# google/layered-scene-inference

Measured on AMD Instinct MI355X. Metric: rendered views/sec (BxLxHxW splat+warp), higher is better.
Workload: dtype f32; 1 GPU; cfg3: 4-layer LDI 256x768, batch 32 per GPU (32 total), trg_downsampling 0.5, kitti cameras, compose_layers, smooth disparities; launch=graph, input_sets_rotated=3, parallelism=batch-sharded replicas x1 (no collective)

## Files before the change

include/lsi_hip.h:

```cpp
#ifndef LSI_HIP_H_
#define LSI_HIP_H_

#include <stddef.h>
#include <stdint.h>

#ifdef __cplusplus
extern "C" {
#endif

#define LSI_VERSION 100

#define LSI_OK 0
#define LSI_EINVAL -1
#define LSI_ENULL -2
#define LSI_EWORKSPACE -3
#define LSI_ELAUNCH -4
#define LSI_EUNSUPPORTED -5

#define LSI_COMPOSE 1u
#define LSI_WANT_DISP 2u
#define LSI_HAS_MASK 4u
#define LSI_WS_KEEP 8u
#define LSI_DETERMINISTIC 16u

// ... 423 lines not shown
#define LSI_FC_X_F32 2u
#define LSI_FC_OUT_F32 4u
typedef struct LsiFcDesc {
  int32_t M, K, N;
  int32_t groups;
  int32_t taps;
  uint32_t flags;
  int64_t w_sn, w_sk;
  int64_t tap_off[4];
  float eps;
  int32_t reserved;
} LsiFcDesc;
size_t lsi_fc_desc_bytes(void);
int lsi_fc_supported(const LsiFcDesc* d);
size_t lsi_fc_workspace_bytes(const LsiFcDesc* d);
int lsi_fc_fwd(const LsiFcDesc* d, const void* x, const float* w, const float* beta, void* y,
               float* z, float* mean_rstd, void* workspace, size_t workspace_bytes,
               lsi_stream_t stream);
int lsi_fc_bwd(const LsiFcDesc* d, const void* x, const float* w, const void* dy,
               const void* y, const float* z, const float* mean_rstd, void* dx, float* dw,
               float* dbeta, void* workspace, size_t workspace_bytes, lsi_stream_t stream);

#define LSI_IMAGE_MAX_PIXELS 16843009
typedef struct LsiImageDesc {
  int64_t offset;
  int32_t H, W, C;
  int32_t reserved;
} LsiImageDesc;
int lsi_area_resize_u8(int32_t n, const LsiImageDesc* desc_host,
                       const LsiImageDesc* desc_dev, const uint8_t* packed,
                       size_t packed_bytes, int32_t Ho, int32_t Wo, int32_t Co,
                       float* out, lsi_stream_t stream);

#ifdef __cplusplus
}
#endif
#endif
```

layered-scene-inference_amd/build.py:

```python
import os
import shutil
import subprocess
import sys

PKG = os.path.dirname(os.path.abspath(__file__))
ROOT = os.path.dirname(PKG)
CSRC = os.path.join(PKG, 'csrc')
SO = os.path.join(PKG, 'liblsi_hip.so')
SOURCES = ['lsi_splat.hip', 'lsi_splat_stream.hip', 'lsi_splat_stream2.hip',
           'lsi_splat_tile.hip', 'lsi_splat_bwd_stream.hip',
           'lsi_splat_sweep.hip',
           'lsi_sampling.hip', 'lsi_loss.hip', 'lsi_eval.hip', 'lsi_bn.hip', 'lsi_host.hip', 'lsi_conv.hip',
           'lsi_conv_wgrad.hip', 'lsi_conv_igemm.hip', 'lsi_conv_wgrad_igemm.hip',
           'lsi_conv_first.hip', 'lsi_conv_f32.hip', 'lsi_scene.hip', 'lsi_fc.hip',
           'lsi_image.hip', 'lsi_ssim.hip', 'lsi_edge_smooth.hip']
HEADERS = [os.path.join(CSRC, 'lsi_common.h'),
           os.path.join(CSRC, 'lsi_layers.h'),
           os.path.join(CSRC, 'lsi_reduce.h'),
           os.path.join(CSRC, 'lsi_splat_internal.h'),
           os.path.join(CSRC, 'lsi_bn_ws.h'),
           os.path.join(CSRC, 'lsi_conv_host.h'),
           os.path.join(CSRC, 'lsi_conv_device.h'),
           os.path.join(ROOT, 'include', 'lsi_hip.h')]

HIPCC_FLAGS = [
    '--offload-arch=gfx950', '-O3', '-std=c++17', '-fPIC',
    '-ffp-contract=off',
    '-munsafe-fp-atomics',
    '-fno-fast-math', '-Wall', '-Wno-unused-function',
]


def hipcc():
  exe = shutil.which('hipcc') or '/opt/rocm/bin/hipcc'
  if not os.path.exists(exe):
    raise RuntimeError('hipcc not found; ROCm toolchain is required')
  return exe


def _stale(target, deps):
  if not os.path.exists(target):
    return True
  t = os.path.getmtime(target)
  return any(os.path.getmtime(d) > t for d in deps)


SO_HOOKS = os.path.join(PKG, 'liblsi_hip_hooks.so')
LAST_BUILD = {}
# ... 41 lines not shown
```

layered-scene-inference_amd/lsi/_C.py:

```python
import ctypes
import os

import torch

_PKG = os.path.dirname(os.path.dirname(os.path.abspath(__file__)))
SO_PATH = os.path.join(_PKG, 'liblsi_hip_%s.so' % os.environ['LSI_HIP_LIB'] if
                       os.environ.get('LSI_HIP_LIB') else 'liblsi_hip.so')

LSI_OK = 0
LSI_COMPOSE, LSI_WANT_DISP, LSI_HAS_MASK, LSI_WS_KEEP = 1, 2, 4, 8
LSI_DETERMINISTIC = 16
LSI_PACKED_RGBD = 32
LSI_GRAD_M = 64
LSI_PATH_AUTO, LSI_PATH_ATOMIC, LSI_PATH_ROWBAND, LSI_PATH_STREAM = 0, 1, 2, 3
LSI_PATH_TILE = 4
LSI_SCENE_IMG, LSI_SCENE_DISP, LSI_SCENE_IMG_ROOM, LSI_SCENE_DISP_ROOM = 1, 2, 4, 8
LSI_SCENE_MAX_PLANES = 16
LSI_FC_BN, LSI_FC_X_F32, LSI_FC_OUT_F32 = 1, 2, 4
LSI_IMAGE_MAX_PIXELS = 16843009
PATH_NAMES = {1: 'atomic', 2: 'rowband', 3: 'stream', 4: 'tile'}

_c_f = ctypes.POINTER(ctypes.c_float)
_c_i = ctypes.POINTER(ctypes.c_int32)

# ... 40 lines not shown


class LsiEdgeSmoothDesc(ctypes.Structure):
  _fields_ = (
      [(n, ctypes.c_int32) for n in ('L', 'B', 'H', 'W', 'order', 'normalise')] +
      [(n, ctypes.c_int64) for n in ('d_sl', 'd_sb', 'd_sy', 'd_sx',
                                     'g_sl', 'g_sb', 'g_sy', 'g_sx', 'g_sc')] +
      [(n, ctypes.c_float) for n in ('alpha', 'eps')])


class LsiConvDesc(ctypes.Structure):
  _fields_ = [(n, ctypes.c_int32) for n in (
      'N', 'H', 'W', 'Cin', 'OH', 'OW', 'Cout', 'KH', 'KW', 'stride', 'pad_t', 'pad_l')]


class LsiSceneDesc(ctypes.Structure):
  _fields_ = ([(n, ctypes.c_int32) for n in ('B', 'V', 'P', 'Hs', 'Ws', 'H', 'W',
                                             'n_box', 'soft')] +
              [('min_disp', ctypes.c_float), ('temp', ctypes.c_float),
               ('outputs', ctypes.c_uint32)])


class LsiFcDesc(ctypes.Structure):
  _fields_ = ([(n, ctypes.c_int32) for n in ('M', 'K', 'N', 'groups', 'taps')] +
              [('flags', ctypes.c_uint32), ('w_sn', ctypes.c_int64),
               ('w_sk', ctypes.c_int64), ('tap_off', ctypes.c_int64 * 4),
               ('eps', ctypes.c_float), ('reserved', ctypes.c_int32)])


class LsiPackJob(ctypes.Structure):
  _fields_ = ([('w', ctypes.c_void_p), ('dst', ctypes.c_void_p)] +
              [(n, ctypes.c_int32) for n in ('D0', 'D1', 'khw', 'tr', 'ntaps', 'block0')] +
              [('tap', ctypes.c_int8 * 56)])


class LsiConvIO(ctypes.Structure):
  _fields_ = ([(n, ctypes.c_void_p) for n in ('x', 'x2', 'packed', 'out', 'out2',
                                              'bn_workspace', 'workspace')] +
              [('workspace_bytes', ctypes.c_size_t), ('c1', ctypes.c_int32),
               ('groups', ctypes.c_int32)])


class LsiImageDesc(ctypes.Structure):
  _fields_ = ([('offset', ctypes.c_int64)] +
              [(n, ctypes.c_int32) for n in ('H', 'W', 'C', 'reserved')])


_I32, _I64, _VP, _SZ = ctypes.c_int32, ctypes.c_int64, ctypes.c_void_p, ctypes.c_size_t
_DP = ctypes.POINTER(LsiSplatDesc)
_LP = ctypes.POINTER(LsiLossDesc)
_CP = ctypes.POINTER(LsiConvDesc)
_F32 = ctypes.c_float
SIGNATURES = {
    'lsi_version': (ctypes.c_int, []),
    'lsi_strerror': (ctypes.c_char_p, [ctypes.c_int]),
    'lsi_bg_weight': (ctypes.c_float, [ctypes.c_double] * 3),
    'lsi_rowband_ok': (ctypes.c_int, [_DP, _VP]),
    'lsi_stream_ok': (ctypes.c_int, [_DP, _VP]),
    'lsi_splat_workspace_bytes': (_SZ, [_DP]),
    'lsi_stream_adapt_state': (ctypes.c_int, [ctypes.POINTER(LsiStreamAdapt)]),
    'lsi_splat_fwd': (ctypes.c_int, [_DP] + [_VP] * 8 + [_SZ, _VP]),
    'lsi_splat_bwd_workspace_bytes': (_SZ, [_DP]),
    'lsi_splat_bwd': (ctypes.c_int, [_DP] + [_VP] * 12 + [_SZ, _VP]),
    'lsi_splat_bwd_m': (ctypes.c_int, [_DP] + [_VP] * 13 + [_SZ, _VP]),
    'lsi_splat_bwd_disp_workspace_bytes': (_SZ, [_DP]),
    'lsi_splat_bwd_disp': (ctypes.c_int, [_DP] + [_VP] * 15 + [_SZ, _VP]),
# ... 68 lines not shown
    'lsi_conv2d_bwd_data_cat': (ctypes.c_int, [_CP, _VP, _VP, _VP, _VP, _I32, _VP]),
    'lsi_conv2d_wgrad_cat': (ctypes.c_int, [_CP, _VP, _VP, _I32, _VP, _VP, _I32, _VP, _SZ, _VP]),
    'lsi_conv2d_workspace_bytes': (_SZ, [_CP, _I32]),
    'lsi_conv2d_run': (ctypes.c_int, [_CP, _I32, ctypes.POINTER(LsiConvIO), _VP]),
    'lsi_conv2d_wgrad_workspace_bytes': (_SZ, [_CP]),
    'lsi_conv2d_wgrad': (ctypes.c_int, [_CP] + [_VP] * 4 + [_SZ, _VP]),
    'lsi_conv2d_first_supported': (ctypes.c_int, [_CP]),
    'lsi_conv2d_first_fwd': (ctypes.c_int, [_CP, _VP, _I32, _VP, _I32, _VP, _VP, _I32, _VP]),
    'lsi_conv2d_first_wgrad_workspace_bytes': (_SZ, [_CP]),
    'lsi_conv2d_first_wgrad': (ctypes.c_int, [_CP, _VP, _I32, _VP, _VP, _I32, _VP, _SZ, _VP]),
    'lsi_conv2d_f32_supported': (ctypes.c_int, [_CP]),
    'lsi_conv2d_f32_packed_bytes': (_SZ, [_CP]),
    'lsi_conv2d_f32_pack': (ctypes.c_int, [_CP, _I32, _VP, _VP, _SZ, _VP]),
    'lsi_conv2d_f32_pack_job': (ctypes.c_int, [_CP, _I32, _VP, _VP, _SZ,
                                               ctypes.POINTER(LsiPackJob), _c_i]),
    'lsi_conv2d_f32_pack_many': (ctypes.c_int, [_VP, _I32, _I32, _VP]),
    'lsi_conv2d_f32_workspace_bytes': (_SZ, [_CP, _I32]),
    'lsi_conv2d_f32_run': (ctypes.c_int, [_CP, _I32, ctypes.POINTER(LsiConvIO), _VP]),
    'lsi_conv2d_wgrad_f32_workspace_bytes': (_SZ, [_CP]),
    'lsi_conv2d_wgrad_f32': (ctypes.c_int, [_CP, _VP, _VP, _I32, _VP, _VP, _I32, _VP, _SZ,
                                            _VP]),
    'lsi_bn_workspace_floats': (_SZ, [_I64, _I32, _I32, _I32]),
    'lsi_bn_relu_fwd': (ctypes.c_int, [_VP] * 5 + [_I64, _I32, _I32, _I32, _F32, _I32, _VP]),
    'lsi_bn_relu_bwd': (ctypes.c_int, [_VP] * 7 + [_I64, _I32, _I32, _I32, _I32, _VP]),
    'lsi_bn_relu_norm': (ctypes.c_int, [_VP] * 5 + [_I64, _I32, _I32, _I32, _F32, _I32, _VP]),
    'lsi_bn_stats_discard': (ctypes.c_int, [_VP, _I32, _VP]),
    'lsi_fc_desc_bytes': (_SZ, []),
    'lsi_fc_supported': (ctypes.c_int, [ctypes.POINTER(LsiFcDesc)]),
    'lsi_fc_workspace_bytes': (_SZ, [ctypes.POINTER(LsiFcDesc)]),
    'lsi_fc_fwd': (ctypes.c_int, [ctypes.POINTER(LsiFcDesc)] + [_VP] * 7 + [_SZ, _VP]),
    'lsi_fc_bwd': (ctypes.c_int, [ctypes.POINTER(LsiFcDesc)] + [_VP] * 10 + [_SZ, _VP]),
    'lsi_area_resize_u8': (ctypes.c_int, [_I32, _VP, _VP, _VP, _SZ] + [_I32] * 3 +
                           [_VP, _VP]),
}

_lib = None


def lib():
  global _lib
  if _lib is None:
    if not os.path.exists(SO_PATH):
      raise RuntimeError(
          'liblsi_hip.so is missing (%s). Build it with '
          '`python layered-scene-inference_amd/build.py`; there is no CPU or '
          'PyTorch fallback for the lsi HIP ops.' % SO_PATH)
    handle = ctypes.CDLL(SO_PATH)
    for name, (res, args) in SIGNATURES.items():
      fn = getattr(handle, name)
      fn.restype = res
      fn.argtypes = args
    _lib = handle
  return _lib


def check(rc, what):
  if rc != LSI_OK:
    msg = lib().lsi_strerror(rc).decode()
    raise RuntimeError('%s failed: %s (code %d)' % (what, msg, rc))


def require_device(*tensors):
  dev = None
  for t in tensors:
    if t is None:
      continue
# ... 34 lines not shown
```

layered-scene-inference_amd/lsi/nnutils/_hip_conv.py:

```python
import os
import torch

from lsi import _C


def supported(x, cin, cout, k, stride, pred):
  if not (x.is_cuda and x.dim() == 4 and x.dtype == torch.bfloat16):
    return False
  if k != 3 or stride != 1 or cin != 32 or x.shape[1] != 32 or x.shape[3] % 16:
    return False
  if pred:
    if not 1 <= cout <= 4:
      return False
  elif cout not in (16, 32):
    return False
  return (x.is_contiguous(memory_format=torch.channels_last) and
          x.data_ptr() % 16 == 0)


def _launch(x, weight, cout, mode, bias=None):
  n, _, h, w = x.shape
  dev = x.device
  weight = _f32(weight)
  if mode == 1:
# ... 314 lines not shown

_PACKED = {}
_PACK_TABLE = {}


def _pack_layout(w):
  if w.dtype == torch.float32:
    if w.is_contiguous():
      return 0
    if w.dim() == 4 and w.is_contiguous(memory_format=torch.channels_last):
      return 2
  return None


def _pack_source(weight):
  w = weight.detach()
  cl = _pack_layout(w)
  if cl is None:
    return w.float().contiguous(), 0
  return w, cl


_HOOK = [None]
PACK_CHECK = int(os.environ.get('LSI_PACK_CHECK', '0'))
_CHECK_CALLS = [0]


def _install_optimizer_hook():
  if _HOOK[0] is None:
    from torch.optim.optimizer import register_optimizer_step_post_hook
    _HOOK[0] = register_optimizer_step_post_hook(_after_optimizer_step)


def _after_optimizer_step(optimizer, args, kwargs):
  del args, kwargs
  if not _PACKED:
    return
  owned = set()
  for group in optimizer.param_groups:
    for p in group['params']:
      owned.add(id(p))
  if any(k[0] in owned for k in _PACKED):
    repack_all(_owned=owned)


def _packed(desc, mode, weight, training=False, dtype=torch.bfloat16):
  key = (id(weight), mode, dtype)
  hit = _PACKED.get(key)
  training = training and weight.requires_grad
  if training:
    _install_optimizer_hook()
  if training and not (hit is not None and hit.managed):
    _PACKED.pop((id(weight), 1 - mode, dtype), None)
    hit_ok = False
  else:
    hit_ok = True
  geo = (desc.Cin, desc.Cout, desc.KH, desc.KW, desc.stride, desc.pad_t, desc.pad_l)
  if hit is not None and hit.wref() is weight and hit.buf.device == weight.device:
    if hit_ok and hit.version == weight._version and hit.geo == geo:
      if PACK_CHECK and hit.managed:
        _CHECK_CALLS[0] += 1
        if _CHECK_CALLS[0] % PACK_CHECK == 0:
          _verify_pack(hit, weight)
      return hit.buf
  lib = _C.lib()
  dev = weight.device
  p = _PRECISIONS[dtype]
  esz = p.esz
  nbytes = getattr(lib, p.packed_bytes)(ctypes.byref(desc))
  if (hit is not None and hit.wref() is weight and hit.buf.device == dev and
      hit.buf.numel() * esz == nbytes and hit.geo == geo):
    buf = hit.buf
  else:
    buf = torch.empty((nbytes // esz,), dtype=dtype, device=dev)
  src, cl = _pack_source(weight)
  rc = getattr(lib, p.pack)(ctypes.byref(desc), mode | cl, _C.ptr(src), _C.ptr(buf),
                            nbytes, _C.stream_ptr(dev))
  _C.check(rc, p.pack)
  e = _Pack()
  e.wref = weakref.ref(weight, lambda _r, k=key: _PACKED.pop(k, None))
  e.version = weight._version
  e.geo = geo
  e.buf, e.mode, e.desc = buf, mode, desc
  e.dtype = dtype
  e.managed = False
  _PACKED[key] = e
  return buf


def _verify_pack(e, weight):
  src, cl = _pack_source(weight)
  fresh = torch.empty_like(e.buf)
  pack = _PRECISIONS[e.dtype].pack
  rc = getattr(_C.lib(), pack)(ctypes.byref(e.desc), e.mode | cl, _C.ptr(src), _C.ptr(fresh),
                               fresh.numel() * fresh.element_size(), _C.stream_ptr(weight.device))
  _C.check(rc, pack)
  if not torch.equal(fresh, e.buf):
    raise RuntimeError('stale packed weights: a %s parameter was updated behind the '
                       'optimiser hook and the version counter (a write through .data?); '
                       'call _hip_conv.repack_all() after such updates'
                       % (tuple(weight.shape),))


def repack_all(device=None, _owned=None):
  if not _PACKED:
    return 0
  lib = _C.lib()
  by_dev = {}
  for k, e in list(_PACKED.items()):
    w = e.wref()
    if w is None:
      continue
    if _owned is not None and k[0] not in _owned:
      continue
    if not w.is_cuda or _pack_layout(w) is None:
      if device is None or w.device == device:
        _PACKED.pop(k, None)
      continue
    if device is not None and w.device != device:
      continue
    if not w.requires_grad and e.version == w._version:
      continue
    by_dev.setdefault((w.device.index, e.dtype), []).append((e, w))
  n = 0
  for (idx, dtype), items in by_dev.items():
    p = _PRECISIONS[dtype]
    key = tuple((w.data_ptr(), e.buf.data_ptr(), e.mode) for e, w in items)
    tabs = _PACK_TABLE.setdefault(idx if dtype == torch.bfloat16 else (idx, dtype), {})
    tab = tabs.get(key)
    if tab is None:
      jobs = (_C.LsiPackJob * len(items))()
      nb = ctypes.c_int32(0)
      blocks = 0
      for j, (e, w) in enumerate(items):
        rc = getattr(lib, p.pack_job)(ctypes.byref(e.desc), e.mode | _pack_layout(w), w.data_ptr(),
                                  e.buf.data_ptr(), e.buf.numel() * e.buf.element_size(),
                                  ctypes.byref(jobs[j]), ctypes.byref(nb))
        _C.check(rc, p.pack_job)
        jobs[j].block0 = blocks
        blocks += nb.value
      host = torch.frombuffer(bytearray(bytes(jobs)), dtype=torch.uint8)
      tab = (key, host.to(items[0][1].device), len(items), blocks)
      tabs[key] = tab
    dev = items[0][1].device
    with torch.cuda.device(dev):
      rc = getattr(lib, p.pack_many)(tab[1].data_ptr(), tab[2], tab[3], _C.stream_ptr(dev))
# ... 363 lines not shown
```

layered-scene-inference_amd/lsi/nnutils/train_utils.py:

```python
import glob
import json
import os
import time

import torch


def define_default_flags(parser):
  a = parser.add_argument
  a('--checkpoint_dir', default='cachedir/snapshots/')
  a('--pretrain_name', default='')
  a('--pretrain_iter', type=int, default=100000)
  a('--batch_size', type=int, default=2)
  a('--num_iter', type=int, default=100000)
  a('--img_height', type=int, default=256)
  a('--img_width', type=int, default=256)
  a('--log_freq', type=int, default=5)
  a('--checkpoint_freq', type=int, default=50000)
  a('--save_latest_freq', type=int, default=2000)
  a('--learning_rate', type=float, default=0.0001)
  a('--beta1', type=float, default=0.9)
  return parser


# ... 28 lines not shown
    use_gpu = torch.cuda.is_available() and not getattr(opts, 'cpu', False)
    if use_gpu:
      torch.cuda.set_device(self.local_rank)
      self.device = torch.device('cuda', self.local_rank)
      torch.backends.cudnn.benchmark = bool(getattr(opts, 'miopen_search', False))
      if getattr(opts, 'miopen_tune', False):
        os.environ.setdefault('MIOPEN_FIND_ENFORCE', '3')
    if self.world > 1 or (getattr(opts, 'flat_grads', False) and
                          'RANK' in os.environ and 'MASTER_ADDR' in os.environ):
      import torch.distributed as dist
      if not dist.is_initialized():
        dist.init_process_group(backend or ('nccl' if use_gpu else 'gloo'))
      self.dist = dist
    torch.manual_seed(0)
    self.define_data_loader()
    self.model = self.build_model().to(self.device)
    if getattr(opts, 'channels_last', False):
      self.model = self.model.to(memory_format=torch.channels_last)
      if use_gpu:
        from lsi.nnutils import nets
        nets.own_kernel_param_layouts(self.model)
    self.train_model = self.model
    self.use_graph = bool(getattr(opts, 'hip_graph', False)) and use_gpu
    self.flat_grads = bool(getattr(opts, 'flat_grads', False)) or \
        (self.use_graph and self.world > 1)
    if self.world > 1 and not self.flat_grads:
      from torch.nn.parallel import DistributedDataParallel as DDP
      self.train_model = DDP(
          self.model, device_ids=[self.local_rank] if use_gpu else None,
          bucket_cap_mb=25, gradient_as_bucket_view=True)
    self._graph, self._graph_plan, self._static = None, None, None
    self._graph_b = None
    self._graph_warm = 0
    self.optim = torch.optim.Adam(self.model.parameters(),
                                  lr=opts.learning_rate,
                                  betas=(opts.beta1, 0.999), eps=1e-8,
                                  capturable=self.use_graph,
                                  fused=bool(use_gpu) and bool(getattr(opts, 'fused_adam', True)))
    if self.use_graph:
      self._stream = torch.cuda.Stream(self.device)
    if use_gpu:
      from lsi.nnutils import _hip_conv
      env = os.environ.get('LSI_WGRAD_STREAM', '')
      _hip_conv.enable_wgrad_stream(
          self.world == 1 and not self.flat_grads and
          (env == '1' or (env != '0' and not self.use_graph)))
      from lsi.nnutils import nets
      env = os.environ.get('LSI_HEAD_STREAMS', '')
      nets.enable_head_streams(
          self.world == 1 and not self.flat_grads and
          (env == '1' or (env != '0' and not self.use_graph)))
      if getattr(opts, 'fp32_convs', None) is not None:
        nets.F32_CONV = opts.fp32_convs == 'own'
    self.resume()
    if self.flat_grads:
      self._setup_flat_grads()

  def _setup_flat_grads(self):
    params = [p for p in self.model.parameters() if p.requires_grad]
    if self.dist is not None and self.world > 1:
      for p in params:
        self.dist.broadcast(p.data, src=0)
    n = sum(p.numel() for p in params)
    self._flat = torch.zeros((n,), dtype=params[0].dtype, device=self.device)
    off = 0
    for p in params:
      p.grad = torch.as_strided(self._flat, p.size(), p.stride(),
                                storage_offset=off)
      off += p.numel()

  def _reduce_flat(self):
# ... 53 lines not shown
      return
    os.makedirs(self.opts.checkpoint_dir, exist_ok=True)
    path = os.path.join(self.opts.checkpoint_dir, name)
    torch.save({'model': self.model.state_dict(),
                'global_step': self.global_step}, path)
    numbered = sorted(glob.glob(os.path.join(self.opts.checkpoint_dir,
                                             'model-*')),
                      key=os.path.getmtime)
    for old in numbered[:-10]:
      os.remove(old)

  def _grad_part(self, staged):
    if self.flat_grads:
      self._flat.zero_()
    else:
      self.optim.zero_grad(set_to_none=True)
    total, scalars = self.compute_losses(staged)
    total.backward()
    return total, scalars

  def _eager_step(self, staged):
    out = self._grad_part(staged)
    if self.flat_grads:
      self._reduce_flat()
    self.optim.step()
    self._after_update()
    return out

  def _after_update(self):
    """Nothing to do: the convolution kernels' packed weights follow the
    parameters through torch.optim's global post-step hook
    (_hip_conv._install_optimizer_hook: one lsi_conv2d_pack_many launch right
    after `optim.step()`, eagerly or inside the captured graph) -- any training
    loop gets that, not only this one."""

  def train_step(self):
    batch = self.feed()
    staged, plan = self.stage(batch)
    if not self.use_graph:
      out = self._eager_step(staged)
    else:
      out = self._graph_step(staged, plan)
    self.global_step += 1
    return out

  GRAPH_WARMUP = 3

  def _graph_step(self, staged, plan):
    cur = torch.cuda.current_stream(self.device)
    if self._graph is not None and plan == self._graph_plan:
      for dst, src in zip(self._static, staged):
        dst.copy_(src)
      return self._replay()
    self._stream.wait_stream(cur)
    with torch.cuda.stream(self._stream):
      if self._graph_warm < self.GRAPH_WARMUP:
        out = self._eager_step(staged)
        self._graph_warm += 1
      else:
        self._graph = None
        self._static = [t.clone() for t in staged]
        self._graph_plan = plan
        if not self.flat_grads:
          self.optim.zero_grad(set_to_none=True)
          graph = torch.cuda.CUDAGraph()
          with torch.cuda.graph(graph, stream=self._stream,
                                capture_error_mode='thread_local'):
# ... 49 lines not shown
```

Before: 396,100 views/s.

## Fuse Adam update with bf16 conv weight packing in one HIP kernel

Adds a custom HIP Adam optimizer, PackingAdam, that updates parameters, moments and steps in a single multi-tensor kernel. For conv weights it also writes the bf16 packed weight layouts straight from the updated values through a shared-memory transpose tile. This removes the separate torch fused-Adam launch plus the post-step lsi_conv2d_pack_many pass that re-read all weights. In exchange it adds a job table, host-side planning and caching logic, and double-precision moment maths that may be slower per element.

```diff
diff --git a/include/lsi_hip.h b/include/lsi_hip.h
--- a/include/lsi_hip.h
+++ b/include/lsi_hip.h
@@ -479,6 +479,29 @@
                        size_t packed_bytes, int32_t Ho, int32_t Wo, int32_t Co,
                        float* out, lsi_stream_t stream);
 
+#define LSI_ADAM_FLAT 0
+#define LSI_ADAM_CONV 1
+typedef struct LsiAdamJob {
+  float* p;
+  const float* g;
+  float* m;
+  float* v;
+  float* step;
+  void* dst[2];
+  int64_t n;
+  int32_t D0, D1, khw, cl, block0, kind;
+  float step_size, bc2_sqrt;
+  int8_t pos[2][56];
+} LsiAdamJob;
+int lsi_adam_job_flat(int64_t n, float* p, const float* g, float* m, float* v, float* step,
+                      LsiAdamJob* job, int32_t* nblocks);
+int lsi_adam_job_conv(const LsiConvDesc* d, int32_t channels_last, float* p, const float* g,
+                      float* m, float* v, float* step, void* packed0, void* packed1,
+                      size_t packed_bytes, LsiAdamJob* job, int32_t* nblocks);
+int lsi_adam_pack_step(LsiAdamJob* jobs_device, const LsiAdamJob* jobs_pinned,
+                       const float* const* grads, int32_t njobs, int32_t total_blocks, double lr,
+                       double beta1, double beta2, double eps, lsi_stream_t stream);
+
 #ifdef __cplusplus
 }
 #endif
diff --git a/layered-scene-inference_amd/build.py b/layered-scene-inference_amd/build.py
--- a/layered-scene-inference_amd/build.py
+++ b/layered-scene-inference_amd/build.py
@@ -13,7 +13,7 @@
            'lsi_sampling.hip', 'lsi_loss.hip', 'lsi_eval.hip', 'lsi_bn.hip', 'lsi_host.hip', 'lsi_conv.hip',
            'lsi_conv_wgrad.hip', 'lsi_conv_igemm.hip', 'lsi_conv_wgrad_igemm.hip',
            'lsi_conv_first.hip', 'lsi_conv_f32.hip', 'lsi_scene.hip', 'lsi_fc.hip',
-           'lsi_image.hip', 'lsi_ssim.hip', 'lsi_edge_smooth.hip']
+           'lsi_image.hip', 'lsi_ssim.hip', 'lsi_edge_smooth.hip', 'lsi_optim.hip']
 HEADERS = [os.path.join(CSRC, 'lsi_common.h'),
            os.path.join(CSRC, 'lsi_layers.h'),
            os.path.join(CSRC, 'lsi_reduce.h'),
diff --git a/layered-scene-inference_amd/csrc/lsi_optim.hip b/layered-scene-inference_amd/csrc/lsi_optim.hip
--- /dev/null
+++ b/layered-scene-inference_amd/csrc/lsi_optim.hip
@@ -0,0 +1,364 @@
+#include <hip/hip_runtime.h>
+#include <math.h>
+#include <stdint.h>
+#include <string.h>
+
+#include "../../include/lsi_hip.h"
+#include "lsi_conv_host.h"
+
+namespace {
+
+constexpr int OPT_TC = 16;
+constexpr int OPT_PITCH = 34;
+constexpr int OPT_TAP = 32 * OPT_PITCH + 2;
+constexpr int OPT_FLAT = 4096;
+
+struct AdamK {
+  double beta1, beta2, eps;
+};
+
+__device__ __forceinline__ void adam_element(const AdamK& k, float step_size, float bc2_sqrt,
+                                             float& p, float g, float& m, float& v) {
+  const double gd = (double)g;
+  m = (float)(k.beta1 * (double)m + (1.0 - k.beta1) * gd);
+  v = (float)(k.beta2 * (double)v + ((1.0 - k.beta2) * gd) * gd);
+  const float denom = (float)((double)(__fsqrt_rn(v) / bc2_sqrt) + k.eps);
+  p = p - (step_size * m) / denom;
+}
+
+constexpr int OPT_CHUNK = 256;
+struct GradPtrs {
+  const float* g[OPT_CHUNK];
+};
+__global__ __launch_bounds__(256) void adam_advance_kernel(LsiAdamJob* jobs, int njobs,
+                                                           GradPtrs gp, int has_g, double lr,
+                                                           double beta1, double beta2) {
+  const int j = (int)threadIdx.x;
+  if (j >= njobs) return;
+  LsiAdamJob& a = jobs[j];
+  if (has_g) a.g = gp.g[j];
+  const float step = *a.step + 1.0f;
+  *a.step = step;
+  const double s = (double)step;
+  const float bc1 = (float)(1.0 - pow(beta1, s));
+  const double bc2 = 1.0 - pow(beta2, s);
+  a.step_size = (float)(lr / (double)bc1);
+  a.bc2_sqrt = (float)sqrt(bc2);
+}
+
+__device__ __forceinline__ void adam_flat(const LsiAdamJob& a, int lb, const AdamK& k) {
+  const float ss = a.step_size, bs = a.bc2_sqrt;
+  float* __restrict__ const p = a.p;
+  const float* __restrict__ const g = a.g;
+  float* __restrict__ const m = a.m;
+  float* __restrict__ const v = a.v;
+  const int64_t n = a.n;
+  const int tid = threadIdx.x;
+  const unsigned lo = (unsigned)((uintptr_t)p & 15);
+  const bool vec = lo == ((uintptr_t)g & 15) && lo == ((uintptr_t)m & 15) &&
+                   lo == ((uintptr_t)v & 15) && (lo & 3) == 0;
+  if (!vec) {
+    const int64_t e0 = (int64_t)lb * OPT_FLAT;
+#pragma unroll 4
+    for (int i = 0; i < OPT_FLAT / 256; ++i) {
+      const int64_t e = e0 + i * 256 + tid;
+      if (e < n) {
+        float pp = p[e], mm = m[e], vv = v[e];
+        adam_element(k, ss, bs, pp, g[e], mm, vv);
+        p[e] = pp; m[e] = mm; v[e] = vv;
+      }
+    }
+    return;
+  }
+  int64_t head = ((16 - lo) & 15) >> 2;
+  if (head > n) head = n;
+  if (lb == 0 && tid < head) {
+    float pp = p[tid], mm = m[tid], vv = v[tid];
+    adam_element(k, ss, bs, pp, g[tid], mm, vv);
+    p[tid] = pp; m[tid] = mm; v[tid] = vv;
+  }
+  const int64_t e0 = head + (int64_t)lb * OPT_FLAT;
+  typedef float f4 __attribute__((ext_vector_type(4)));
+  for (int i0 = 0; i0 < 4; i0 += 2) {
+    f4 P[2], G[2], M[2], V[2];
+#pragma unroll
+    for (int i = 0; i < 2; ++i) {
+      const int64_t e = e0 + (int64_t)((i0 + i) * 256 + tid) * 4;
+      if (e + 4 <= n) {
+        P[i] = *reinterpret_cast<const f4*>(p + e);
+        G[i] = *reinterpret_cast<const f4*>(g + e);
+        M[i] = *reinterpret_cast<const f4*>(m + e);
+        V[i] = *reinterpret_cast<const f4*>(v + e);
+      }
+    }
+#pragma unroll
+    for (int i = 0; i < 2; ++i) {
+      const int64_t e = e0 + (int64_t)((i0 + i) * 256 + tid) * 4;
+      if (e + 4 <= n) {
+#pragma unroll
+        for (int c = 0; c < 4; ++c) {
+          float pp = P[i][c], mm = M[i][c], vv = V[i][c];
+          adam_element(k, ss, bs, pp, G[i][c], mm, vv);
+          P[i][c] = pp; M[i][c] = mm; V[i][c] = vv;
+        }
+        *reinterpret_cast<f4*>(p + e) = P[i];
+        *reinterpret_cast<f4*>(m + e) = M[i];
+        *reinterpret_cast<f4*>(v + e) = V[i];
+      } else if (e < n) {
+        for (int64_t x = e; x < n; ++x) {
+          float pp = p[x], mm = m[x], vv = v[x];
+          adam_element(k, ss, bs, pp, g[x], mm, vv);
+          p[x] = pp; m[x] = mm; v[x] = vv;
+        }
+      }
+    }
+  }
+}
+
+__device__ __forceinline__ void adam_conv_tile(const LsiAdamJob& a, int bx, int by,
+                                               unsigned short* tile, const AdamK& k) {
+  const float ss = a.step_size, bs = a.bc2_sqrt;
+  float* __restrict__ const p = a.p;
+  const float* __restrict__ const g = a.g;
+  float* __restrict__ const m = a.m;
+  float* __restrict__ const v = a.v;
+  const int D0 = a.D0, D1 = a.D1, khw = a.khw;
+  const bool cl = a.cl != 0;
+  const int a0 = by * 32, b0 = bx * 32;
+  const int nr = min(32, D0 - a0), nc = min(32, D1 - b0);
+  const int tid = threadIdx.x, lane = tid & 63, wave = tid >> 6;
+  const size_t per = (size_t)D0 * D1;
+  typedef float f4 __attribute__((ext_vector_type(4)));
+  const bool al16 = !(((uintptr_t)p | (uintptr_t)g | (uintptr_t)m | (uintptr_t)v) & 15);
+  unsigned short* const dst0 = reinterpret_cast<unsigned short*>(a.dst[0]);
+  unsigned short* const dst1 = reinterpret_cast<unsigned short*>(a.dst[1]);
+  for (int t0 = 0; t0 < khw; t0 += OPT_TC) {
+    const int nt = min(OPT_TC, khw - t0);
+    const unsigned magic = (65536u + nt - 1) / nt;
+    const int len = cl ? 32 * nt : nc * nt;
+    const bool vec = al16 && (cl ? !(D1 & 3) && !(nc & 3)
+                                 : nt == khw && !((D1 * khw) & 3) && !((nc * khw) & 3));
+    if (vec) {
+      const int len4 = len >> 2;
+      const int nchunk = (len4 + 63) >> 6;
+      const int nq = 8 * nchunk;
+      for (int q0 = 0; q0 < nq; q0 += 2) {
+        f4 P[2], G[2], M[2], V[2];
+        size_t off[2];
+        int row[2], i4[2];
+#pragma unroll
+        for (int u = 0; u < 2; ++u) {
+          const int q = q0 + u;
+          const int rr = q / nchunk, ch = q - rr * nchunk;
+          const int r = wave + 4 * rr;
+          i4[u] = ch * 64 + lane;
+          const bool ok = q < nq && r < nr && i4[u] < len4 && (!cl || (i4[u] & 7) * 4 < nc);
+          row[u] = ok ? r : -1;
+          off[u] = cl ? ((size_t)(a0 + r) * khw + t0 + (i4[u] >> 3)) * D1 + b0 + (i4[u] & 7) * 4
+                      : ((size_t)(a0 + r) * D1 + b0) * khw + 4 * i4[u];
+          if (ok) {
+            P[u] = *reinterpret_cast<const f4*>(p + off[u]);
+            G[u] = *reinterpret_cast<const f4*>(g + off[u]);
+            M[u] = *reinterpret_cast<const f4*>(m + off[u]);
+            V[u] = *reinterpret_cast<const f4*>(v + off[u]);
+          }
+        }
+#pragma unroll
+        for (int u = 0; u < 2; ++u) {
+          if (row[u] >= 0) {
+#pragma unroll
+            for (int j = 0; j < 4; ++j) {
+              float pp = P[u][j], mm = M[u][j], vv = V[u][j];
+              adam_element(k, ss, bs, pp, G[u][j], mm, vv);
+              P[u][j] = pp; M[u][j] = mm; V[u][j] = vv;
+              int c, tt;
+              if (cl) { tt = i4[u] >> 3; c = (i4[u] & 7) * 4 + j; }
+              else {
+                const int i = 4 * i4[u] + j;
+                c = (int)(((unsigned)i * magic) >> 16); tt = i - c * nt;
+              }
+              tile[tt * OPT_TAP + row[u] * OPT_PITCH + c] =
+                  __builtin_bit_cast(unsigned short, (__bf16)pp);
+            }
+            *reinterpret_cast<f4*>(p + off[u]) = P[u];
+            *reinterpret_cast<f4*>(m + off[u]) = M[u];
+            *reinterpret_cast<f4*>(v + off[u]) = V[u];
+          }
+        }
+      }
+    }
+    const int nchunk = (len + 63) >> 6;
+    const int nq = vec ? 0 : 8 * nchunk;
+    for (int q0 = 0; q0 < nq; q0 += 4) {
+      float P[4], G[4], M[4], V[4];
+      size_t off[4];
+      int li[4];
+#pragma unroll
+      for (int u = 0; u < 4; ++u) {
+        const int q = q0 + u;
+        const int rr = q / nchunk, ch = q - rr * nchunk;
+        const int r = wave + 4 * rr;
+        const int i = ch * 64 + lane;
+        int c, tt;
+        if (cl) { tt = i >> 5; c = i & 31; }
+        else { c = (int)(((unsigned)i * magic) >> 16); tt = i - c * nt; }
+        const bool ok = q < nq && r < nr && i < len && c < nc;
+        li[u] = ok ? tt * OPT_TAP + r * OPT_PITCH + c : -1;
+        off[u] = cl ? ((size_t)(a0 + r) * khw + t0 + tt) * D1 + b0 + c
+                    : ((size_t)(a0 + r) * D1 + b0 + c) * khw + t0 + tt;
+        if (ok) { P[u] = p[off[u]]; G[u] = g[off[u]]; M[u] = m[off[u]]; V[u] = v[off[u]]; }
+      }
+#pragma unroll
+      for (int u = 0; u < 4; ++u) {
+        if (li[u] >= 0) {
+          adam_element(k, ss, bs, P[u], G[u], M[u], V[u]);
+          p[off[u]] = P[u]; m[off[u]] = M[u]; v[off[u]] = V[u];
+          tile[li[u]] = __builtin_bit_cast(unsigned short, (__bf16)P[u]);
+        }
+      }
+    }
+    __syncthreads();
+    const int cp = 2 * (tid & 15), rb = tid >> 4;
+    for (int tt = 0; tt < nt; ++tt) {
+      const unsigned short* const tl = tile + tt * OPT_TAP;
+#pragma unroll
+      for (int j = 0; j < 2; ++j) {
+        const int r = rb + 16 * j;
+        if (dst0 && r < nr && cp < nc) {
+          unsigned short* const d =
+              dst0 + (size_t)a.pos[0][t0 + tt] * per + (size_t)(a0 + r) * D1 + b0 + cp;
+          const unsigned short x0 = tl[r * OPT_PITCH + cp], x1 = tl[r * OPT_PITCH + cp + 1];
+          if (cp + 1 < nc && !(D1 & 1)) {
+            *reinterpret_cast<unsigned*>(d) = (unsigned)x0 | ((unsigned)x1 << 16);
+          } else {
+            d[0] = x0;
+            if (cp + 1 < nc) d[1] = x1;
+          }
+        }
+        if (dst1 && r < nc && cp < nr) {
+          unsigned short* const d =
+              dst1 + (size_t)a.pos[1][t0 + tt] * per + (size_t)(b0 + r) * D0 + a0 + cp;
+          const unsigned short x0 = tl[cp * OPT_PITCH + r], x1 = tl[(cp + 1) * OPT_PITCH + r];
+          if (cp + 1 < nr && !(D0 & 1)) {
+            *reinterpret_cast<unsigned*>(d) = (unsigned)x0 | ((unsigned)x1 << 16);
+          } else {
+            d[0] = x0;
+            if (cp + 1 < nr) d[1] = x1;
+          }
+        }
+      }
+    }
+    __syncthreads();
+  }
+}
+
+__global__ __launch_bounds__(256, 4) void adam_pack_kernel(const LsiAdamJob* jobs, int njobs,
+                                                        AdamK k) {
+  __shared__ unsigned short tile[OPT_TC * OPT_TAP];
+  int which = -1;
+  for (int j0 = 0; j0 < njobs; j0 += 256) {
+    const int j = j0 + (int)threadIdx.x;
+    which += __syncthreads_count(j < njobs && jobs[j].block0 <= (int)blockIdx.x);
+  }
+  const LsiAdamJob& a = jobs[which];
+  const int lb = (int)blockIdx.x - a.block0;
+  if (a.kind == LSI_ADAM_FLAT) {
+    adam_flat(a, lb, k);
+  } else {
+    const int nbx = (a.D1 + 31) / 32;
+    adam_conv_tile(a, lb % nbx, lb / nbx, tile, k);
+  }
+}
+
+struct TapClass {
+  int ntaps, OHt, OWt, wofs, ooy, oox;
+  signed char tdy[64], tdx[64];
+};
+struct TapArgs {
+  TapClass cls[4];
+  int ncls, N, H, W, Cin, Cout, s, os, OHF, OWF;
+};
+
+}
+
+extern "C" int lsi_adam_job_flat(int64_t n, float* p, const float* g, float* m, float* v,
+                                 float* step, LsiAdamJob* job, int32_t* nblocks) {
+  if (!p || !g || !m || !v || !step || !job || !nblocks) return LSI_ENULL;
+  if (n <= 0 || n > (int64_t)OPT_FLAT * 0x7fffffff) return LSI_EINVAL;
+  if (((uintptr_t)p | (uintptr_t)g | (uintptr_t)m | (uintptr_t)v | (uintptr_t)step) & 3)
+    return LSI_EINVAL;
+  memset(job, 0, sizeof(*job));
+  job->p = p; job->g = g; job->m = m; job->v = v; job->step = step;
+  job->n = n;
+  job->kind = LSI_ADAM_FLAT;
+  *nblocks = (int32_t)((n + 3 + OPT_FLAT - 1) / OPT_FLAT);
+  return LSI_OK;
+}
+
+extern "C" int lsi_adam_job_conv(const LsiConvDesc* d, int32_t channels_last, float* p,
+                                 const float* g, float* m, float* v, float* step, void* packed0,
+                                 void* packed1, size_t packed_bytes, LsiAdamJob* job,
+                                 int32_t* nblocks) {
+  if (!d || !p || !g || !m || !v || !step || !job || !nblocks) return LSI_ENULL;
+  if (d->Cin <= 0 || d->Cout <= 0 || d->KH < 1 || d->KW < 1 || d->KH > 7 || d->KW > 7)
+    return LSI_EINVAL;
+  if (d->stride != 1 && d->stride != 2) return LSI_EINVAL;
+  if (d->pad_t < 0 || d->pad_l < 0 || d->pad_t >= d->KH || d->pad_l >= d->KW) return LSI_EINVAL;
+  if (((uintptr_t)p | (uintptr_t)g | (uintptr_t)m | (uintptr_t)v | (uintptr_t)step) & 3)
+    return LSI_EINVAL;
+  if (((uintptr_t)packed0 | (uintptr_t)packed1) & 15) return LSI_EINVAL;
+  const int khw = d->KH * d->KW;
+  const int64_t tiles = (int64_t)((d->Cin + 31) / 32) * ((d->Cout + 31) / 32);
+  if ((int64_t)d->Cin * d->Cout * khw >= (1ll << 31) || tiles >= (1ll << 31)) return LSI_EINVAL;
+  if ((packed0 || packed1) &&
+      packed_bytes < (size_t)khw * d->Cin * d->Cout * sizeof(uint16_t))
+    return LSI_EWORKSPACE;
+  memset(job, 0, sizeof(*job));
+  job->p = p; job->g = g; job->m = m; job->v = v; job->step = step;
+  job->dst[0] = packed0; job->dst[1] = packed1;
+  job->n = (int64_t)d->Cin * d->Cout * khw;
+  job->D0 = d->Cout; job->D1 = d->Cin; job->khw = khw;
+  job->cl = channels_last ? 1 : 0;
+  job->kind = LSI_ADAM_CONV;  for (int mode = 0; mode < 2; ++mode) {
+    TapArgs k;
+    int8_t tap[64];
+    conv_classes(d, mode, k, tap);
+    for (int t = 0; t < khw; ++t) job->pos[mode][tap[t]] = (int8_t)t;
+  }
+  *nblocks = (int32_t)tiles;
+  return LSI_OK;
+}
+
+extern "C" int lsi_adam_pack_step(LsiAdamJob* jobs_device, const LsiAdamJob* jobs_pinned,
+                                  const float* const* grads, int32_t njobs,
+                                  int32_t total_blocks, double lr, double beta1, double beta2,
+                                  double eps, lsi_stream_t stream_) {
+  if (!jobs_device) return LSI_ENULL;
+  if (njobs <= 0 || total_blocks <= 0) return LSI_EINVAL;
+  if (!(lr >= 0.0) || !(beta1 >= 0.0 && beta1 < 1.0) || !(beta2 >= 0.0 && beta2 < 1.0) ||
+      !(eps >= 0.0))
+    return LSI_EINVAL;
+  if (grads)
+    for (int j = 0; j < njobs; ++j) {
+      if (!grads[j]) return LSI_ENULL;
+      if ((uintptr_t)grads[j] & 3) return LSI_EINVAL;
+    }
+  hipStream_t stream = (hipStream_t)stream_;
+  if (jobs_pinned &&
+      hipMemcpyAsync(jobs_device, jobs_pinned, (size_t)njobs * sizeof(LsiAdamJob),
+                     hipMemcpyHostToDevice, stream) != hipSuccess)
+    return LSI_ELAUNCH;
+  for (int j0 = 0; j0 < njobs; j0 += OPT_CHUNK) {
+    const int n = njobs - j0 < OPT_CHUNK ? njobs - j0 : OPT_CHUNK;
+    GradPtrs gp;
+    memset(&gp, 0, sizeof(gp));
+    if (grads) memcpy(gp.g, grads + j0, (size_t)n * sizeof(gp.g[0]));
+    hipLaunchKernelGGL(adam_advance_kernel, dim3(1), dim3(256), 0, stream, jobs_device + j0, n,
+                       gp, grads ? 1 : 0, lr, beta1, beta2);
+    if (hipGetLastError() != hipSuccess) return LSI_ELAUNCH;
+  }
+  AdamK k = {beta1, beta2, eps};
+  hipLaunchKernelGGL(adam_pack_kernel, dim3(total_blocks), dim3(256), 0, stream,
+                     (const LsiAdamJob*)jobs_device, njobs, k);
+  return hipGetLastError() == hipSuccess ? LSI_OK : LSI_ELAUNCH;
+}
diff --git a/layered-scene-inference_amd/lsi/_C.py b/layered-scene-inference_amd/lsi/_C.py
--- a/layered-scene-inference_amd/lsi/_C.py
+++ b/layered-scene-inference_amd/lsi/_C.py
@@ -96,6 +96,14 @@
   _fields_ = ([('w', ctypes.c_void_p), ('dst', ctypes.c_void_p)] +
               [(n, ctypes.c_int32) for n in ('D0', 'D1', 'khw', 'tr', 'ntaps', 'block0')] +
               [('tap', ctypes.c_int8 * 56)])
+
+
+class LsiAdamJob(ctypes.Structure):
+  _fields_ = ([(n, ctypes.c_void_p) for n in ('p', 'g', 'm', 'v', 'step')] +
+              [('dst', ctypes.c_void_p * 2), ('n', ctypes.c_int64)] +
+              [(n, ctypes.c_int32) for n in ('D0', 'D1', 'khw', 'cl', 'block0', 'kind')] +
+              [('step_size', ctypes.c_float), ('bc2_sqrt', ctypes.c_float),
+               ('pos', ctypes.c_int8 * 112)])
 
 
 class LsiConvIO(ctypes.Structure):
@@ -230,6 +238,10 @@
     'lsi_fc_bwd': (ctypes.c_int, [ctypes.POINTER(LsiFcDesc)] + [_VP] * 10 + [_SZ, _VP]),
     'lsi_area_resize_u8': (ctypes.c_int, [_I32, _VP, _VP, _VP, _SZ] + [_I32] * 3 +
                            [_VP, _VP]),
+    'lsi_adam_job_flat': (ctypes.c_int, [_I64] + [_VP] * 5 + [ctypes.POINTER(LsiAdamJob), _c_i]),
+    'lsi_adam_job_conv': (ctypes.c_int, [_CP, _I32] + [_VP] * 7 +
+                          [_SZ, ctypes.POINTER(LsiAdamJob), _c_i]),
+    'lsi_adam_pack_step': (ctypes.c_int, [_VP, _VP, _VP, _I32, _I32] + [ctypes.c_double] * 4 + [_VP]),
 }
 
 _lib = None
diff --git a/layered-scene-inference_amd/lsi/nnutils/_hip_conv.py b/layered-scene-inference_amd/lsi/nnutils/_hip_conv.py
--- a/layered-scene-inference_amd/lsi/nnutils/_hip_conv.py
+++ b/layered-scene-inference_amd/lsi/nnutils/_hip_conv.py
@@ -370,16 +370,20 @@
     _HOOK[0] = register_optimizer_step_post_hook(_after_optimizer_step)
 
 
+_FRESH = {}
+
+
 def _after_optimizer_step(optimizer, args, kwargs):
   del args, kwargs
+  fresh = _FRESH.pop(id(optimizer), ())
   if not _PACKED:
     return
   owned = set()
   for group in optimizer.param_groups:
     for p in group['params']:
       owned.add(id(p))
-  if any(k[0] in owned for k in _PACKED):
-    repack_all(_owned=owned)
+  if any(k[0] in owned and k not in fresh for k in _PACKED):
+    repack_all(_owned=owned, _skip=fresh)
 
 
 def _packed(desc, mode, weight, training=False, dtype=torch.bfloat16):
@@ -440,7 +444,7 @@
                        % (tuple(weight.shape),))
 
 
-def repack_all(device=None, _owned=None):
+def repack_all(device=None, _owned=None, _skip=()):
   if not _PACKED:
     return 0
   lib = _C.lib()
@@ -449,7 +453,7 @@
     w = e.wref()
     if w is None:
       continue
-    if _owned is not None and k[0] not in _owned:
+    if _owned is not None and (k[0] not in _owned or k in _skip):
       continue
     if not w.is_cuda or _pack_layout(w) is None:
       if device is None or w.device == device:
diff --git a/layered-scene-inference_amd/lsi/nnutils/optim.py b/layered-scene-inference_amd/lsi/nnutils/optim.py
--- /dev/null
+++ b/layered-scene-inference_amd/lsi/nnutils/optim.py
@@ -0,0 +1,205 @@
+import ctypes
+import os
+
+import torch
+
+from lsi import _C
+from lsi.nnutils import _hip_conv
+
+_JOB_BYTES = ctypes.sizeof(_C.LsiAdamJob)
+_JOB_WORDS = _JOB_BYTES // 8
+_PTR = torch.Tensor.data_ptr
+_BF16 = torch.bfloat16
+
+
+def _layout(t):
+  if t.is_contiguous():
+    return 0
+  if t.dim() == 4 and t.is_contiguous(memory_format=torch.channels_last):
+    return 2
+  return None
+
+
+class _Plan(object):
+  __slots__ = ('state', 'group', 'ids', 'mask', 'params', 'ms', 'vs', 'steps', 'layouts',
+               'gstrides', 'dev', 'last_grads', 'geo4')
+
+
+class _Table(object):
+  __slots__ = ('dev', 'host', 'njobs', 'blocks', 'uploaded')
+
+
+class PackingAdam(torch.optim.Adam):
+
+  def _fusable_group(self, group):
+    lr = group['lr']
+    return (group.get('fused') and isinstance(lr, float) and not group['amsgrad'] and
+            not group['maximize'] and group['weight_decay'] == 0 and
+            not group.get('differentiable') and not group.get('foreach'))
+
+  def _torch_step(self, closure):
+    fn = torch.optim.Adam.step
+    if getattr(fn, 'hooked', False):
+      fn = fn.__wrapped__
+    return fn(self, closure)
+
+  def step(self, closure=None):
+    if (os.environ.get('LSI_ADAM_PACK', '1') == '0' or
+        getattr(self, 'grad_scale', None) is not None or
+        getattr(self, 'found_inf', None) is not None or
+        not all(self._fusable_group(g) for g in self.param_groups)):
+      return self._torch_step(closure)
+    self._cuda_graph_capture_health_check()
+    loss = None
+    if closure is not None:
+      with torch.enable_grad():
+        loss = closure()
+    with torch.no_grad():
+      plans = [self._plan(gi, group) for gi, group in enumerate(self.param_groups)]
+      if any(pl is False for pl in plans):
+        return self._torch_step(None) if loss is None else self._torch_step(lambda: loss)
+      fresh = set()
+      for (gi, group), pl in zip(enumerate(self.param_groups), plans):
+        if pl is not None:
+          self._launch(gi, group, pl[0], pl[1], fresh)
+      if fresh and _hip_conv._HOOK[0] is not None:
+        _hip_conv._FRESH[id(self)] = fresh
+    return loss
+
+  def _plan(self, gi, group):
+    cache = self.__dict__.setdefault('_lsi_plans', {})
+    allp = group['params']
+    grads_all = [p.grad for p in allp]
+    mask = tuple([g is not None for g in grads_all])
+    grads = [g for g in grads_all if g is not None]
+    if not grads:
+      return None
+    c = cache.get(gi)
+    if (c is not None and c.state is self.state and c.group is group and c.mask == mask and
+        c.ids == tuple(map(id, allp))):
+      f32, dev = torch.float32, c.dev
+      last = c.last_grads
+      for i, g in enumerate(grads):
+        if g is last[i]:
+          continue
+        if not (g.dtype is f32 and g.layout is torch.strided and g.device == dev and
+                g.stride() == c.gstrides[i]):
+          c = None
+          break
+      if c is not None:
+        c.last_grads = grads
+        return c, grads
+    params, grads, ms, vs, steps = [], [], [], [], []
+    if self._init_group(group, params, grads, ms, vs, [], steps):
+      return False
+    dev = params[0].device
+    layouts = []
+    for p, g, m, v, s in zip(params, grads, ms, vs, steps):
+      for t in (p, g, m, v):
+        if not (t.dtype is torch.float32 and t.is_cuda and t.device == dev and
+                t.layout is torch.strided and t.shape == p.shape):
+          return False
+      if not (s.dtype is torch.float32 and s.is_cuda and s.device == dev and s.numel() == 1):
+        return False
+      lay = _layout(p)
+      if lay is None or any(_layout(t) != lay for t in (g, m, v)):
+        return False
+      layouts.append(lay)
+    c = _Plan()
+    c.state, c.group, c.ids, c.mask = self.state, group, tuple(map(id, allp)), mask
+    c.params, c.ms, c.vs, c.steps, c.layouts, c.dev = params, ms, vs, steps, layouts, dev
+    c.gstrides = [g.stride() for g in grads]
+    c.geo4 = [(p.shape[1], p.shape[0], p.shape[2], p.shape[3]) if p.dim() == 4 else None
+              for p in params]
+    c.last_grads = grads
+    cache[gi] = c
+    return c, grads
+
+  def _packs(self, c):
+    packed = _hip_conv._PACKED
+    out = []
+    for p, geo4 in zip(c.params, c.geo4):
+      if geo4 is None or not packed:
+        out.append(None)
+        continue
+      e0, e1 = packed.get((id(p), 0, _BF16)), packed.get((id(p), 1, _BF16))
+      if e0 is None and e1 is None:
+        out.append(None)
+        continue
+      es = []
+      for e in (e0, e1):
+        if e is not None and not (e.wref() is p and e.buf.device == c.dev and
+                                  e.geo[:4] == geo4):
+          e = None
+        es.append(e)
+      if es[0] is not None and es[1] is not None and es[0].geo != es[1].geo:
+        es[1] = None
+      out.append(tuple(es) if (es[0] is not None or es[1] is not None) else None)
+    return out
+
+  def _build(self, c, grads, packs):
+    lib = _C.lib()
+    n = len(c.params)
+    jobs = (_C.LsiAdamJob * n)()
+    nb = ctypes.c_int32(0)
+    blocks = 0
+    for j in range(n):
+      p, g, m, v, s = c.params[j], grads[j], c.ms[j], c.vs[j], c.steps[j]
+      es = packs[j]
+      if es is None:
+        rc = lib.lsi_adam_job_flat(p.numel(), p.data_ptr(), g.data_ptr(), m.data_ptr(),
+                                   v.data_ptr(), s.data_ptr(), ctypes.byref(jobs[j]),
+                                   ctypes.byref(nb))
+        _C.check(rc, 'lsi_adam_job_flat')
+      else:
+        e = es[0] if es[0] is not None else es[1]
+        bufs = [None if x is None else x.buf for x in es]
+        rc = lib.lsi_adam_job_conv(
+            ctypes.byref(e.desc), c.layouts[j], p.data_ptr(), g.data_ptr(), m.data_ptr(),
+            v.data_ptr(), s.data_ptr(), _C.ptr(bufs[0]), _C.ptr(bufs[1]),
+            e.buf.numel() * e.buf.element_size(), ctypes.byref(jobs[j]), ctypes.byref(nb))
+        _C.check(rc, 'lsi_adam_job_conv')
+      jobs[j].block0 = blocks
+      blocks += nb.value
+    return jobs, blocks
+
+  def _table(self, gi, c, grads, packs):
+    dsts = tuple([0 if es is None else
+                  (0 if es[0] is None else es[0].buf.data_ptr(),
+                   0 if es[1] is None else es[1].buf.data_ptr()) for es in packs])
+    key = (gi, tuple(map(_PTR, c.params)), tuple(map(_PTR, c.ms)), tuple(map(_PTR, c.vs)),
+           tuple(map(_PTR, c.steps)), dsts)
+    tables = self.__dict__.setdefault('_lsi_tables', {})
+    tab = tables.get(key)
+    if tab is None:
+      jobs, blocks = self._build(c, grads, packs)
+      n = len(c.params)
+      tab = tables[key] = _Table()
+      tab.njobs, tab.blocks, tab.uploaded = n, blocks, False
+      tab.host = torch.empty((n, _JOB_WORDS), dtype=torch.int64).pin_memory()
+      tab.host.view(torch.uint8).view(-1).copy_(
+          torch.frombuffer(bytearray(bytes(jobs)), dtype=torch.uint8))
+      tab.dev = torch.empty((n, _JOB_WORDS), dtype=torch.int64, device=c.dev)
+    if tab.uploaded:
+      return tab, None
+    tab.uploaded = not torch.cuda.is_current_stream_capturing()
+    return tab, tab.host
+
+  def _launch(self, gi, group, c, grads, fresh):
+    packs = self._packs(c)
+    beta1, beta2 = group['betas']
+    with torch.cuda.device(c.dev):
+      tab, host = self._table(gi, c, grads, packs)
+      gptrs = (ctypes.c_void_p * tab.njobs)(*map(_PTR, grads))
+      rc = _C.lib().lsi_adam_pack_step(tab.dev.data_ptr(), _C.ptr(host), gptrs, tab.njobs,
+                                       tab.blocks, float(group['lr']), float(beta1),
+                                       float(beta2), float(group['eps']), _C.stream_ptr(c.dev))
+    _C.check(rc, 'lsi_adam_pack_step')
+    for p, es in zip(c.params, packs):
+      if es is None:
+        continue
+      for mode, e in enumerate(es):
+        if e is not None:
+          e.version = p._version
+          e.managed = True
+          fresh.add((id(p), mode, _BF16))
diff --git a/layered-scene-inference_amd/lsi/nnutils/train_utils.py b/layered-scene-inference_amd/lsi/nnutils/train_utils.py
--- a/layered-scene-inference_amd/lsi/nnutils/train_utils.py
+++ b/layered-scene-inference_amd/lsi/nnutils/train_utils.py
@@ -84,11 +84,15 @@
     self._graph, self._graph_plan, self._static = None, None, None
     self._graph_b = None
     self._graph_warm = 0
-    self.optim = torch.optim.Adam(self.model.parameters(),
-                                  lr=opts.learning_rate,
-                                  betas=(opts.beta1, 0.999), eps=1e-8,
-                                  capturable=self.use_graph,
-                                  fused=bool(use_gpu) and bool(getattr(opts, 'fused_adam', True)))
+    adam = torch.optim.Adam
+    if use_gpu:
+      from lsi.nnutils import optim as lsi_optim
+      adam = lsi_optim.PackingAdam
+    self.optim = adam(self.model.parameters(),
+                      lr=opts.learning_rate,
+                      betas=(opts.beta1, 0.999), eps=1e-8,
+                      capturable=self.use_graph,
+                      fused=bool(use_gpu) and bool(getattr(opts, 'fused_adam', True)))
     if self.use_graph:
       self._stream = torch.cuda.Stream(self.device)
     if use_gpu:
@@ -208,7 +212,8 @@
     parameters through torch.optim's global post-step hook
     (_hip_conv._install_optimizer_hook: one lsi_conv2d_pack_many launch right
     after `optim.step()`, eagerly or inside the captured graph) -- any training
-    loop gets that, not only this one."""
+    loop gets that, not only this one.  PackingAdam's fused step writes the bf16
+    packs itself; the hook then has only the rest to pack, usually nothing."""
 
   def train_step(self):
     batch = self.feed()
```

Result: slower. 390,200 views/s (-1.5%).
